# worldlife123/cbench_BaSIC

Hardware: AMD Instinct MI355X
Metric: encode+decode Mpix/s (higher is better)
Workload: dtype f32; 1 GPU; hyperprior codec N=128 M=192 (lossy_graph_scalable_exp_hp), synthetic 3x256x256 images (image i = manual_seed(i), rand), 256 images per GPU per step resident in HBM, compress+decompress incl. bitstream D2H/H2D, 6 concurrent stream workers per GPU (step k on worker k mod W: whole batches, W in flight); images_per_gpu=256, workers=6, rans_waves_per_workgroup=8, batches_in_flight=6, parallelism=image-sharded x1, RCCL all-reduce of metric sums

## Files before the change

cbench_basic_amd/_lib.py:

```python
import ctypes
import os

_HERE = os.path.dirname(os.path.abspath(__file__))
LIB_PATH = os.path.join(_HERE, "libbasic_hip.so")

OK, ERR_INVALID, ERR_NOT_INIT, ERR_HIP, ERR_OVERFLOW, ERR_NO_DEVICE = 0, -1, -2, -3, -4, -5
IMAGE_CHW, IMAGE_HWC = 0, 1
PIXEL_U8, PIXEL_F32 = 0, 1


class BasicHipError(RuntimeError):
    pass


class BasicHipInvalid(BasicHipError, ValueError):
    """A call the library refuses (BASIC_ERR_INVALID / BASIC_ERR_NOT_INIT): a ValueError, as the reference's pybind11 layer
    raises, and like every other failure of the library a BasicHipError."""


_lib = None

c_i32p = ctypes.c_void_p
_I, _L, _P, _F = ctypes.c_int, ctypes.c_int64, ctypes.c_void_p, ctypes.c_float

# ... 39 lines not shown
    "basic_rans_cost_table_host": (_I, [_P, _I, _I, _P, _I, _P]),
    "basic_rans_tables_costs": (_I, [_P, _P]),
    "basic_gc_rate_curve_dev": (_I, [_P, _P, _I, _L, _I, _P, _I, _I, _P, _I, _F, _P, _P, _P]),
    "basic_gc_quantize_index_ms_dev": (_I, [_P, _P, _P, _L, _L, _L, _P, _I, _P, _I, _F, _P, _P, _P, _P]),
    "basic_gc_dequantize_ms_dev": (_I, [_P, _P, _L, _L, _L, _P, _I, _P, _P]),
    "basic_gc_rate_curve_ms_dev": (_I, [_P, _P, _P, _L, _I, _L, _I, _P, _I, _I, _P, _I, _F, _P, _P, _P]),
    "basic_rate_select_dev": (_I, [_P, _I, _I, _L, _P, _I, _I, _P, _P, _P, _P, _P, _P]),
    "basic_rate_refine_dev": (_I, [_P, _I, _I, _P, _I, _P, _P, _P]),
    "basic_rate_select_groups_dev": (_I, [_P, _I, _I, _I, _P, _P, _P, _I, _P, _P, _P, _P, _I, _I, _P, _P, _P, _P, _P, _P, _I, _P]),
    "basic_hp_session_set_rate_targets": (_I, [_P, _P, _I, _P, _I, _I]),
    "basic_hp_session_rate_result": (_I, [_P, _P, _P, _P, _I]),
    "basic_eb_quantize_index_dev": (_I, [_P, _P, _I, _I, _I, _P, _P, _P, _P]),
    "basic_eb_dequantize_dev": (_I, [_P, _P, _I, _I, _I, _P, _P]),
    "basic_i32_to_f32_dev": (_I, [_P, _L, _P, _P]),
    "basic_pgm_gauss_encode_group_dev": (_I, [_P, _P, _I, _I, _I, _P, _L, _P, _I, _P, _P, _L, _L, _P, _P]),
    "basic_pgm_gauss_index_group_dev": (_I, [_P, _I, _I, _I, _P, _L, _P, _I, _P, _L, _L, _P]),
    "basic_pgm_gauss_scatter_group_dev": (_I, [_P, _P, _I, _I, _I, _P, _L, _L, _L, _P, _P]),
    "basic_gauss_nll_per_image_dev": (_I, [_P, _P, _I, _I, _I, _I, _F, _F, _P, _P]),
    "basic_gauss_nll_per_image_q_dev": (_I, [_P, _P, _I, _I, _I, _P, _I, _F, _F, _P, _P]),
    "basic_eb_nll_per_image_dev": (_I, [_P, _P, _I, _I, _I, _F, _P, _P]),
    "basic_conv_plan_create": (_I, [_P, _P, _I, _I, _I, _I, _I, _I, _I, _I, _P, _P, _I, _I, _P]),
    "basic_conv_plan_out_hw": (_I, [_P, _I, _I, _P, _P]),
    "basic_conv_forward_dev": (_I, [_P, _P, _I, _I, _I, _P, _P]),
    "basic_conv_plan_channels": (_I, [_P, _P, _P]),
    "basic_hp_session_create": (_I, [_P, _I, _P, _I, _P, _I, _P, _I, _P, _I, _P, _P, _I, _F, _P, _P]),
    "basic_hp_encode_bound": (_L, [_P, _I, _I, _I]),
    "basic_hp_encode_images": (_I, [_P, _P, _I, _I, _I, _I, _P, _L, _P, _P]),
    "basic_hp_encode_result": (_I, [_P, _P, _L, _P]),
    "basic_hp_decoded_shape": (_I, [_P, _P, _L, _P, _P, _P, _P]),
    "basic_hp_decode_images": (_I, [_P, _P, _L, _P, _L, _P]),
    "basic_image_u8_to_f32_dev": (_I, [_P, _I, _I, _I, _I, _I, _P, _P]),
    "basic_image_f32_to_u8_dev": (_I, [_P, _I, _I, _I, _I, _I, _P, _P]),
    "basic_image_sse_u8_dev": (_I, [_P, _I, _P, _I, _I, _I, _I, _I, _P, _P]),
    "basic_image_tiles_u8_to_f32_dev": (_I, [_P, _I, _I, _I, _I, _I, _I, _I, _I, _I, _I, _I, _I, _P, _P]),
    "basic_image_tiles_f32_to_u8_dev": (_I, [_P, _I, _I, _I, _I, _I, _I, _I, _I, _I, _I, _I, _P, _I, _I, _I, _P]),
    "basic_image_tiles_overlap_u8_to_f32_dev": (_I, [_P, _I, _I, _I, _I, _I, _I, _I, _I, _I, _I, _I, _I, _P, _P]),
    "basic_image_tiles_blend_dev": (_I, [_P, _I, _I, _I, _I, _I, _I, _I, _I, _I, _I, _I, _P, _I, _I, _P]),
    "basic_image_tiles_last_path": (_I, [_P]),
    "basic_image_tiles_gather_u8_to_f32_dev": (_I, [_P, _I, _I, _I, _I, _P, _P, _P]),
    "basic_image_tiles_scatter_f32_to_u8_dev": (_I, [_P, _I, _I, _I, _I, _I, _P, _I, _P, _P]),
    "basic_image_tiles_gather_pad_u8_to_f32_dev": (_I, [_P, _I, _I, _I, _I, _P, _P, _P]),
    "basic_image_tiles_scatter_clip_f32_to_u8_dev": (_I, [_P, _I, _I, _I, _I, _I, _P, _I, _P, _P]),
    "basic_hp_encode_images_u8": (_I, [_P, _P, _I, _I, _I, _I, _I, _P, _L, _P, _P]),
    "basic_hp_decode_images_u8": (_I, [_P, _P, _L, _I, _P, _I, _L, _P]),
    "basic_hp_session_set_rans_waves": (_I, [_P, _I]),
    "basic_hp_session_set_stream_lanes": (_I, [_P, _I]),
# ... 95 lines not shown
```

cbench_basic_amd/csrc/conv.hip:

```cpp
#include "common.h"

#include <algorithm>
#include <cmath>
#include <cstdlib>
#include <cstring>
#include <new>
#include <vector>

using namespace basic;

namespace {
thread_local bool g_dynamic_tiles = false;
}
namespace basic {
bool set_dynamic_tiles(bool on)
{
    const bool prev = g_dynamic_tiles;
    g_dynamic_tiles = on;
    return prev;
}
}

namespace {

// ... 401 lines not shown

__global__ __launch_bounds__(256) void image_absmax_kernel(const float *x, int64_t n, int per_img, unsigned *amax)
{
    const int img = blockIdx.x / per_img, part = blockIdx.x - img * per_img;
    const float *src = x + img * n;
    unsigned m = 0;
    if (((reinterpret_cast<uintptr_t>(src) | static_cast<uintptr_t>(n * 4)) & 15) == 0) {
        const u32x4 *s4 = reinterpret_cast<const u32x4 *>(src);
        for (int64_t i = part * 256 + threadIdx.x; i < n / 4; i += per_img * 256) {
            const u32x4 v = s4[i];
#pragma unroll
            for (int e = 0; e < 4; ++e) m = max(m, v[e] & 0x7FFFFFFFu);
        }
    } else {
        for (int64_t i = part * 256 + threadIdx.x; i < n; i += per_img * 256) m = max(m, __float_as_uint(src[i]) & 0x7FFFFFFFu);
    }
#pragma unroll
    for (int off = 32; off > 0; off >>= 1) m = max(m, static_cast<unsigned>(__shfl_xor(static_cast<int>(m), off)));
    if ((threadIdx.x & 63) == 0 && m) atomicMax(amax + img, m);
}

constexpr int kSplitPatchPos = 416;
constexpr int kSplitPieceBytes = kSplitPatchPos * 32;
constexpr size_t kSplitLdsPatchBytes = kSplitLdsBytes + 2 * kSplitPieceBytes;
static_assert(kSplitLdsPatchBytes <= 160 * 1024, "patch beside the weight stages");
static_assert(kSplitLdsBytes % 16 == 0, "16-byte aligned patch");
constexpr int kSplitPatchRounds = (2 * kSplitPatchPos + kSplitThreads - 1) / kSplitThreads;

template <int KH, int KW, int KWB, bool PATCH>
__global__ __launch_bounds__(kSplitThreads, 1) void conv_split_f16_kernel(const TapLaunch g, const u32x4 *wsplit, const int *kw,
                                                                          const unsigned *amax)
{
    constexpr int MT = 4;
    constexpr int kTapsA = KH * KW, kTapsAll = KH * (KW + KWB);
    constexpr int kGroups = kTapsAll / kSplitStageTaps;
    static_assert(kTapsAll % kSplitStageTaps == 0, "taps per channel block must be whole stages");
    static_assert(KWB > 0 && KWB <= KW, "fused phases: second grid inside the first");
    extern __shared__ u32x4 lds_u4[];
    float *chan_const = reinterpret_cast<float *>(lds_u4 + 2 * kSplitStageU4);

    const int tid = threadIdx.x;
    const int lane = tid & 63;
    const int khalf = lane >> 5;
    const int wave = __builtin_amdgcn_readfirstlane(tid >> 6);

    int bid = xcd_tile(blockIdx.x, gridDim.x);
    const int tx_i = bid % g.tiles_x; bid /= g.tiles_x;
    const int ty_i = bid % g.tiles_y; bid /= g.tiles_y;
    const int TB = 1 << g.tb_log, TH = 1 << g.th_log, TW = 1 << g.tw_log;
    const int b0 = bid * TB, my0 = ty_i * TH, mx0 = tx_i * TW;
    struct Pos { int tb, my, mx; };
    auto pos_of = [&](int t) {
        const int qq = (t >> 6) * 32 + (t & 31);
        return Pos{qq >> (g.tw_log + g.th_log), my0 + ((qq >> g.tw_log) & (TH - 1)), mx0 + (qq & (TW - 1))};
// ... 62 lines not shown
    if constexpr (PATCH) {
#pragma unroll
        for (int r = 0; r < kSplitPatchRounds; ++r) {
            const int i = r * kSplitThreads + tid, p = i >> 1, h = i & 1;
            const int prow = p / PW, x = p - prow * PW, img = prow / PH, row = prow - img * PH;
            const int gy = my0 + g.dymin + row, gx = mx0 + g.dxmin + x;
            const bool inside = i < 2 * npos && img < nimg && gy >= 0 && gy < g.in_h && gx >= 0 && gx < g.in_w;
            pvoff[r] = inside ? static_cast<int>((((static_cast<int64_t>(img) * g.cin + 8 * h) * g.in_h + gy) * g.in_w + gx) * 4)
                              : 0x7FFFFFF0;
            pkx[r] = inside ? split_act_exp(amax[b0 + img]) : 0;
        }
#pragma unroll
        for (int dy = 0; dy < KH; ++dy) brow[dy] = ((tb * PH + (lp.my - my0) + dy) * PW + (lp.mx - mx0)) * 32 + 16 * khalf;
    }
    float pf[kSplitPatchRounds][8];
    auto fetch_patch = [&](int cb) __attribute__((always_inline)) {
        const int soff = cb * kSplitCK * plane_bytes;
#pragma unroll
        for (int r = 0; r < kSplitPatchRounds; ++r)
#pragma unroll
            for (int j = 0; j < 8; ++j)
                pf[r][j] = __builtin_bit_cast(float, __builtin_amdgcn_raw_buffer_load_b32(rsrc, pvoff[r], soff + j * plane_bytes, 0));
    };
    auto store_patch = [&]() __attribute__((always_inline)) {
#pragma unroll
        for (int r = 0; r < kSplitPatchRounds; ++r)
            if (r * kSplitThreads + tid < 2 * npos) {
                u32x4 q[2];
                split_f16x2(pf[r], pkx[r], q[0], q[1]);
#pragma unroll
                for (int pc = 0; pc < 2; ++pc)
                    *reinterpret_cast<u32x4 *>(patch + (r * kSplitThreads + tid) * 16 + pc * kSplitPieceBytes) = q[pc];
            }
    };
    auto read_b = [&](int T, u32x4 (&d)[2]) __attribute__((always_inline)) {
        const char *src = patch + brow[tap_row(T)] + 32 * tap_col(T);
#pragma unroll
        for (int pc = 0; pc < 2; ++pc) d[pc] = *reinterpret_cast<const u32x4 *>(src + pc * kSplitPieceBytes);
    };

    f32x16 acc[MT], acc2[MT];
#pragma unroll
    for (int m = 0; m < MT; ++m)
#pragma unroll
        for (int r = 0; r < 16; ++r) {
            acc[m][r] = 0.f;
            acc2[m][r] = 0.f;
        }

    float xb[8];
    u32x4 bq[2][2];
    if constexpr (PATCH) fetch_patch(0);
    else load_b(0, 0, xb);
    fetch_w(0, 0);
    store_w(0, 0);
    fetch_w(0, 1);
    store_w(0, 1);
    if constexpr (PATCH) store_patch();
    for (int cb = 0; cb < ncb; ++cb) {
#pragma unroll
        for (int gi = 0; gi < kGroups; ++gi) {
            const int s = cb * kGroups + gi;
            __syncthreads();
            const bool more = s + 1 < ncb * kGroups;
            if (more) fetch_w(s + 1, 0);
            __builtin_amdgcn_sched_barrier(0);
            const u32x4 *wl = lds_u4 + (s & 1) * kSplitStageU4 + lane;
#pragma unroll
            for (int tl = 0; tl < kSplitStageTaps; ++tl) {
                const int T = gi * kSplitStageTaps + tl;
                float xn[8];
                u32x4 bd[2];
                if constexpr (PATCH) {
                    if (T == 0) read_b(0, bq[0]);
                } else {
                    if (T + 1 < kTapsAll) load_b(cb, T + 1, xn);
                    else load_b(cb + 1 < ncb ? cb + 1 : cb, 0, xn);
                    __builtin_amdgcn_sched_barrier(0);
                    split_f16x2(xb, kx_l, bd[0], bd[1]);
                }
                const u32x4 (&bp)[2] = PATCH ? bq[T & 1] : bd;
// ... 14 lines not shown
                        if (m == MT - 3 && T + 1 < kTapsAll) read_b(T + 1, bq[(T + 1) & 1]);
                    }
                    __builtin_amdgcn_sched_barrier(0);
                    dst[m] = mfma_f16(ap[cur][1], bp[0], dst[m]);
                    dst[m] = mfma_f16(ap[cur][0], bp[1], dst[m]);
                    dst[m] = mfma_f16(ap[cur][0], bp[0], dst[m]);
                    __builtin_amdgcn_sched_barrier(0);
                }
                if constexpr (!PATCH) {
#pragma unroll
                    for (int j = 0; j < 8; ++j) xb[j] = xn[j];
                }
                if (tl == 1 && more) {
                    store_w((s + 1) & 1, 0);
                    fetch_w(s + 1, 1);
                    __builtin_amdgcn_sched_barrier(0);
                }
                if constexpr (PATCH) {
                    if (gi == 0 && tl == 1) {
                        fetch_patch(cb + 1 < ncb ? cb + 1 : cb);
                        __builtin_amdgcn_sched_barrier(0);
                    }
                }
                if (tl == 3 && more) store_w((s + 1) & 1, 1);
            }
        }
        if constexpr (PATCH) {
            if (cb + 1 < ncb) {
                __syncthreads();
                store_patch();
            }
        }
    }

    const int tid_e = wave * 64 + static_cast<int>(__lane_id());
    const int khalf_e = (tid_e >> 5) & 1, col_e = tid_e & 31;
    float *gl = reinterpret_cast<float *>(lds_u4);
    const bool gdn = g.act == BASIC_ACT_GDN || g.act == BASIC_ACT_IGDN;
    const int be_s = b0 + pos_of(tid_e).tb;
    const int kx_e = be_s < g.batch ? split_act_exp(amax[be_s]) : 0;
    auto finish = [&](f32x16 (&acc)[MT]) __attribute__((always_inline)) {
#pragma unroll
        for (int m = 0; m < MT; ++m)
#pragma unroll
            for (int rq = 0; rq < 4; ++rq) {
                const i32x4 k4 = *reinterpret_cast<const i32x4 *>(chan_const + 256 + 32 * m + 8 * rq + 4 * khalf_e);
#pragma unroll
                for (int e = 0; e < 4; ++e) acc[m][4 * rq + e] = __builtin_ldexpf(acc[m][4 * rq + e], -(k4[e] + kx_e));
            }
        if (g.bias) {
#pragma unroll
            for (int m = 0; m < MT; ++m)
#pragma unroll
                for (int rq = 0; rq < 4; ++rq) {
// ... 26 lines not shown
                    const f32x4 b4 = *reinterpret_cast<const f32x4 *>(chan_const + 128 + 32 * m + 8 * rq + 4 * khalf_e);
#pragma unroll
                    for (int e = 0; e < 4; ++e) {
                        const int r = 4 * rq + e;
                        const float nv = nrm[m][r] + b4[e];
                        acc[m][r] *= (g.act == BASIC_ACT_GDN) ? __builtin_amdgcn_rsqf(nv) : __builtin_amdgcn_sqrtf(nv);
                    }
                }
        }
    };
    if (gdn) {
        __syncthreads();
        const f32x4 *src = reinterpret_cast<const f32x4 *>(g.gammaT);
        f32x4 *dst = reinterpret_cast<f32x4 *>(gl);
#pragma unroll
        for (int sl = 0; sl < 128 * 32 * 4 / 4 / kSplitThreads; ++sl) dst[sl * kSplitThreads + tid_e] = src[sl * kSplitThreads + tid_e];
        __syncthreads();
    }
    finish(acc);
    finish(acc2);

    const Pos ep = pos_of(tid_e);
    const int my = ep.my, mx = ep.mx, be = b0 + ep.tb;
    if (my < g.mh && mx < g.mw && be < g.batch) {
        const int oy = my * g.s_out + g.oy0, ox = mx * g.s_out + g.ox0;
        const int64_t oplane = static_cast<int64_t>(g.out_h) * g.out_w;
        float *o = g.out + (static_cast<int64_t>(be) * g.out_ctotal + g.co_base) * oplane + static_cast<int64_t>(oy) * g.out_w + ox;
#pragma unroll
        for (int m = 0; m < MT; ++m)
#pragma unroll
            for (int r = 0; r < 16; ++r) {
                const int co = 32 * m + 8 * (r >> 2) + 4 * khalf_e + (r & 3);
                if (co < g.cout) {
                    f32x2 v2;
                    v2[0] = apply_act(acc[m][r], g.act);
                    v2[1] = apply_act(acc2[m][r], g.act);
                    *reinterpret_cast<f32x2 *>(o + co * oplane) = v2;
                }
            }
    }
}

template <int KH, bool PATCH>
hipError_t launch_split(const TapLaunch &g, const u32x4 *ws, const int *kw, const unsigned *amax, int blocks, hipStream_t st)
{
    const hipError_t e = ensure_max_lds(reinterpret_cast<const void *>(conv_split_f16_kernel<KH, 3, 2, PATCH>));
    if (e != hipSuccess) return e;
    hipLaunchKernelGGL((conv_split_f16_kernel<KH, 3, 2, PATCH>), dim3(blocks), dim3(kSplitThreads),
                       PATCH ? kSplitLdsPatchBytes : kSplitLdsBytes, st, g, ws, kw, amax);
    return hipGetLastError();
}

constexpr int kFirstSlots = 10;

template <bool ROWS>
__global__ __launch_bounds__(512, 1) void conv5x5_cin4_gdn_persistent_kernel(const TapLaunch g, int ntiles, int *sched)
{
    extern __shared__ float lds[];
    constexpr int MT = 4, kCK = ROWS ? 3 : 4, KW = 5, kSteps = ROWS ? 5 * 8 : 25 * 2;
    constexpr int kWFloats = ROWS ? 80 * 32 * 4 : 25 * 4 * 32 * 4;
    constexpr int kGFloats = 128 * 32 * 4;
    float *wl = lds;
    float *gl = lds + kWFloats;
    const int tid = threadIdx.x;
    const int lane = tid & 63;
    const int wave = __builtin_amdgcn_readfirstlane(tid >> 6);
    const int khalf = lane >> 5, col = lane & 31;
    const int TB = 1 << g.tb_log, TH = 1 << g.th_log, TW = 1 << g.tw_log;
    const int chan_stride = g.ph * g.pwp;
    const int patch_elems = TB * kCK * chan_stride;
    const int patch_pad = (patch_elems + 511) / 512 * 512;
    const int n_pslots = patch_pad / 512;
// ... 949 lines not shown
    const bool two_strips = dma_ok && in_h >= 64;
    const int tile_h = two_strips ? SmTile<2>::kTileH : SmTile<1>::kTileH;
    g.tiles_y = (in_h + tile_h - 1) / tile_h;
    g.tiles_x = (in_w + kSmTileW - 1) / kSmTileW;
    const dim3 grid(batch * g.tiles_y * g.tiles_x);
    if (two_strips) hipLaunchKernelGGL(deconv5s2_cout3_dma_kernel<2>, grid, dim3(256), 0, st, g);
    else if (dma_ok) hipLaunchKernelGGL(deconv5s2_cout3_dma_kernel<1>, grid, dim3(256), 0, st, g);
    else hipLaunchKernelGGL(deconv5s2_cout3_kernel, grid, dim3(256), 0, st, g);
    BASIC_HIP_TRY(hipGetLastError());
    return BASIC_OK;
}
}

extern "C" int basic_conv_plan_launches(const basic_conv_plan *p, int batch, int in_h, int in_w)
{
    int oh = 0, ow = 0;
    if (!p || batch < 1 || basic_conv_plan_out_hw(p, in_h, in_w, &oh, &ow)) return -1;
    if (p->d_wsm) return 1;
    int n = 0;
    for_each_launch(p, choose_launches(p, batch, oh, ow, nullptr), oh, ow, [&](const Chunk &, const Phase &, int, int) { ++n; return BASIC_OK; });
    return n;
}

extern "C" int basic_conv_forward_dev(const basic_conv_plan *p, const float *d_in, int batch, int in_h, int in_w,
                                      float *d_out, void *hip_stream)
{
    BASIC_REQUIRE(p && d_in && d_out && batch >= 1, "conv_forward: bad argument");
    int oh = 0, ow = 0;
    int rc = basic_conv_plan_out_hw(p, in_h, in_w, &oh, &ow);
    if (rc) return rc;
    if (p->d_wsm) return launch_small_deconv(p, d_in, batch, in_h, in_w, d_out, as_stream(hip_stream));
    const LaunchChoice choice = choose_launches(p, batch, oh, ow, d_out);
    bool amax_done = false;
    return for_each_launch(p, choice, oh, ow, [&](const Chunk &ch, const Phase &ph, int mh, int mw) -> int {
        TapLaunch g{};
        g.in = d_in; g.out = d_out; g.wpack = ph.d_wpack; g.wrow = ph.d_wrow; g.split_wstride = ph.split_wstride; g.bias = ch.d_bias; g.gammaT = p->d_gammaT; g.beta = p->d_beta;
        g.batch = batch; g.cin = p->cin; g.cin_pad = ph.ntaps ? ph.cin_pad : 0; g.cout = ch.cout; g.coutp = ch.coutp; g.out_ctotal = p->cout; g.co_base = ch.co0;
        g.in_h = in_h; g.in_w = in_w; g.out_h = oh; g.out_w = ow;
        g.s_in = p->s_in; g.s_out = p->s_out; g.oy0 = ph.oy0; g.ox0 = ph.ox0;
        g.mh = mh; g.mw = mw;
        g.ntaps = ph.ntaps; g.dymin = ph.dymin; g.dxmin = ph.dxmin;
        std::memcpy(g.dy, ph.dy, sizeof(g.dy));
        std::memcpy(g.dx, ph.dx, sizeof(g.dx));
        g.act = p->act;
        const int kCK = ph.ck;
        if (choice.split_f16 && ph.d_wsplit) {
            const TileShape ts = tile_shape(g.mh, g.mw, kSplitWaves * 32);
            const int tw = ts.tw, th = ts.th, tb = ts.tb;
            if (static_cast<int64_t>(tb) * p->cin * in_h * in_w * 4 < (1ll << 31)) {
                g.tw_log = ilog2(tw); g.th_log = ilog2(th); g.tb_log = ilog2(tb);
                g.tiles_y = (g.mh + th - 1) / th;
                g.tiles_x = (g.mw + tw - 1) / tw;
                const int blocks = ((batch + tb - 1) / tb) * g.tiles_y * g.tiles_x;
                hipStream_t st = as_stream(hip_stream);
                const u32x4 *ws = static_cast<const u32x4 *>(ph.d_wsplit);
                BASIC_REQUIRE(ph.kw == 3 && ph.kwb == 2 && (ph.kh == 3 || ph.kh == 2), "conv_forward: split-fp16 plan / kernel instantiation mismatch");
                if (!amax_done) {
                    auto *pm = const_cast<basic_conv_plan *>(p);
                    if (pm->amax_cap < batch) {
                        if (pm->d_amax) BASIC_HIP_TRY(hipFree(pm->d_amax));
                        pm->d_amax = nullptr; pm->amax_cap = 0;
                        BASIC_HIP_TRY(hipMalloc(&pm->d_amax, sizeof(unsigned) * batch));
                        pm->amax_cap = batch;
                    }
                    BASIC_HIP_TRY(hipMemsetAsync(pm->d_amax, 0, sizeof(unsigned) * batch, st));
                    const int64_t n = static_cast<int64_t>(p->cin) * in_h * in_w;
                    const int per_img = static_cast<int>(std::min<int64_t>(64, std::max<int64_t>(1, n / 4096)));
                    hipLaunchKernelGGL(image_absmax_kernel, dim3(batch * per_img), dim3(256), 0, st, d_in, n, per_img, pm->d_amax);
                    BASIC_HIP_TRY(hipGetLastError());
                    amax_done = true;
                }
                const bool patch = choice.split_patch && g.s_in == 1 && tb * (th + ph.kh - 1) * (tw + ph.kw - 1) <= kSplitPatchPos;
                const unsigned *am = p->d_amax;
                const hipError_t e = ph.kh == 3 ? (patch ? launch_split<3, true>(g, ws, ph.d_wsplit_k, am, blocks, st) : launch_split<3, false>(g, ws, ph.d_wsplit_k, am, blocks, st))
                                                : (patch ? launch_split<2, true>(g, ws, ph.d_wsplit_k, am, blocks, st) : launch_split<2, false>(g, ws, ph.d_wsplit_k, am, blocks, st));
                BASIC_HIP_TRY(e);
                return BASIC_OK;
            }
        }
        const int threads = 64 * ph.waves, tile_pos = 32 * ph.waves;
        const TileShape ts = tile_shape(g.mh, g.mw, tile_pos);
        const int tw = ts.tw;
        int th = ts.th, tb = ts.tb;
        const bool first_layer_path = ch.mt == 4 && ch.nsplit == 1 && ph.waves == 8 && ph.kh == 5 && ph.kw == 5 &&
                                      ph.cin_pad == kCK && kCK == 4 && ch.cout == 128 && p->d_gammaT;
        g.ph = (th - 1) * g.s_in + ph.span_y;
        g.pw = (tw - 1) * g.s_in + ph.span_x;
        g.patch4 = (ph.waves == 8 && !first_layer_path && in_w % 4 == 0 && (reinterpret_cast<uintptr_t>(d_in) & 15) == 0) ? 1 : 0;
        g.pwp = g.patch4 ? (g.pw + 3 + 3) / 4 * 4 : (g.pw | 1);
        int punit = g.patch4 ? 4 : 1;
        const int mtp = mtile_pitch(ch.mt);
        const int wl_floats = g.ntaps * kCK * 32 * mtp, gam_floats = 32 * 32 * mtp;
        const int wl_pad = ((wl_floats > gam_floats ? wl_floats : gam_floats) + 4 * threads - 1) / (4 * threads) * (4 * threads);
        auto patch_slots_needed = [&](int tbv) { return (tbv * kCK * g.ph * g.pwp / punit + threads - 1) / threads; };
        auto lds_need = [&](int tbv) {
            const int patch_pad = ((tbv * kCK * g.ph * g.pwp / punit + 63) & ~63) * punit;
            return sizeof(float) * (2 * static_cast<size_t>(wl_pad + patch_pad) + 32 + 2 * g.coutp);
        };
        const int slots_avail = ph.kwb ? kPSlotsFused : patch_slots(ch.mt);
        auto too_large = [&](int tbv) { return patch_slots_needed(tbv) > slots_avail || lds_need(tbv) > 160 * 1024; };
        while (tb > 1 && too_large(tb)) tb >>= 1;
// ... 65 lines not shown
```

cbench_basic_amd/csrc/session.hip:

```cpp
#include "common.h"

#include <cstring>
#include <map>
#include <mutex>
#include <vector>

using namespace basic;

constexpr int kMaxTokenLanes = 4;


namespace {

struct DBuf {
    void *p = nullptr;
    size_t cap = 0;
    int ensure(size_t bytes)
    {
        if (bytes <= cap) return BASIC_OK;
        if (p) (void)hipFree(p);
        p = nullptr;
        cap = 0;
        const size_t want = bytes + bytes / 4 + 256;
        BASIC_HIP_TRY(hipMalloc(&p, want));
// ... 73 lines not shown
struct basic_hp_session {
    std::vector<const basic_conv_plan *> g_a, h_a, h_s, g_s;
    const basic_rans_tables *z_tables = nullptr, *y_tables = nullptr;
    int z_channels = 0, y_channels = 0, x_channels = 0, out_channels = 0, n_scales = 0;
    float scale_bound = 0.11f;
    bool mean_scale = false;
    int rans_waves = 0;
    int lanes = 1;
    int res_lanes = 1;
    std::vector<float> qsteps;
    HBuf h_steps;
    DBuf d_steps;
    hipEvent_t steps_done = nullptr;
    std::vector<int64_t> rate_budget;
    std::vector<float> rate_cand;
    int rate_passes = 0, rate_res_batch = 0;
    HBuf h_rate, h_rate_out;
    DBuf d_rate_in, d_rate_bits, d_rate_cand[2], d_rate_out;
    hipEvent_t rate_up = nullptr;
    int skip_rows = 0;
    DBuf skip_scratch, y_symc, y_idxc;
    DBuf d_medians, d_table;
    DBuf act[2], d_x, d_y, d_z, d_zhat, d_prior, d_scales;
    DBuf z_sym, z_idx, y_sym, y_idx, seg_z, seg_y, slots_z, slots_y, nw, off, packed, words, woff, state, pos;
    HBuf h_nw, h_words, h_in;
    std::vector<int64_t> off_z, off_y;
    int res_batch = 0, res_zh = 0, res_zw = 0, res_yh = 0, res_yw = 0;
    hipEvent_t in_done = nullptr;
    hipStream_t side = nullptr;
    hipEvent_t fork = nullptr, join = nullptr;
    bool use_token = false;
    int token_lanes = 0;
    hipEvent_t enc_phase = nullptr, dec_phase = nullptr;
    hipStream_t copy = nullptr;
    hipEvent_t x_free = nullptr, x_ready = nullptr;
    bool x_read_pending = false;
    DBuf u8_in, u8_out, d_xhat;
    hipEvent_t u8_free = nullptr, xhat_free = nullptr;
    bool u8_read_pending = false, xhat_read_pending = false;
    ~basic_hp_session();
};

namespace {

int run_chain(basic_hp_session *s, const std::vector<const basic_conv_plan *> &plans, const float *d_in, int batch, int h, int w,
              DBuf *out_buf, float *d_final, int *oh_out, int *ow_out, hipStream_t st)
{
    const float *cur = d_in;
    int flip = 0;
    for (size_t i = 0; i < plans.size(); ++i) {
        int oh = 0, ow = 0, co = 0;
        int rc = basic_conv_plan_out_hw(plans[i], h, w, &oh, &ow);
        if (rc) return rc;
        rc = basic_conv_plan_channels(plans[i], nullptr, &co);
        if (rc) return rc;
        const size_t bytes = sizeof(float) * static_cast<size_t>(batch) * co * oh * ow;
        float *dst;
        if (i + 1 == plans.size()) {
            if (d_final) dst = d_final;
            else { rc = out_buf->ensure(bytes); if (rc) return rc; dst = out_buf->as<float>(); }
        } else {
            rc = s->act[flip].ensure(bytes);
            if (rc) return rc;
            dst = s->act[flip].as<float>();
            flip ^= 1;
        }
        rc = basic_conv_forward_dev(plans[i], cur, batch, h, w, dst, st);
        if (rc) return rc;
        cur = dst;
        h = oh;
        w = ow;
    }
    if (oh_out) *oh_out = h;
    if (ow_out) *ow_out = w;
    return BASIC_OK;
}

int chain_out_hw(const std::vector<const basic_conv_plan *> &plans, int h, int w, int *oh, int *ow)
{
    for (const auto *p : plans) {
        int a = 0, b = 0;
        int rc = basic_conv_plan_out_hw(p, h, w, &a, &b);
        if (rc) return rc;
        h = a;
        w = b;
    }
    *oh = h;
    *ow = w;
    return BASIC_OK;
}

// ... 829 lines not shown
```

cbench_basic_amd/nn/kernels.py:

```python
import contextlib
import ctypes
import os

import numpy as np
import torch

from .. import _lib

ACT_NONE, ACT_RELU, ACT_LEAKY_RELU, ACT_GDN, ACT_IGDN = 0, 1, 2, 3, 4


def _dev(t, dtype=None):
    if not isinstance(t, torch.Tensor) or not t.is_cuda:
        raise _lib.BasicHipError("cbench_basic_amd kernels need tensors on the MI355X (got a CPU tensor); "
                                 "there is no CPU fallback")
    if dtype is not None and t.dtype != dtype:
        raise TypeError(f"expected {dtype}, got {t.dtype}")
    return t.contiguous()


def _stream():
    return torch.cuda.current_stream().cuda_stream


# ... 23 lines not shown
            int(output_padding), int(self.transposed), int(act), g.ctypes.data if g is not None else None,
            be.ctypes.data if be is not None else None, self.cin, self.cout, ctypes.byref(h)))
        self._h = h

    def __del__(self):
        h, self._h = getattr(self, "_h", None), None
        if h:
            try:
                _lib.lib().basic_conv_plan_destroy(h)
            except Exception:
                pass

    def out_hw(self, h, w):
        oh, ow = ctypes.c_int(), ctypes.c_int()
        _lib.check(_lib.lib().basic_conv_plan_out_hw(self._h, int(h), int(w), ctypes.byref(oh), ctypes.byref(ow)))
        return oh.value, ow.value

    def flops(self, batch, h, w):
        return int(_lib.lib().basic_conv_plan_flops(self._h, int(batch), int(h), int(w)))

    def launches(self, batch, h, w):
        return int(_lib.lib().basic_conv_plan_launches(self._h, int(batch), int(h), int(w)))

    def __call__(self, x, out=None):
        x = _dev(x, torch.float32)
        B, C, H, W = x.shape
        if C != self.cin:
            raise ValueError(f"conv plan expects {self.cin} input channels, got {C}")
        oh, ow = self.out_hw(H, W)
        if out is None:
            out = torch.empty((B, self.cout, oh, ow), device=x.device, dtype=torch.float32)
        _lib.check(_lib.lib().basic_conv_forward_dev(self._h, x.data_ptr(), B, H, W, out.data_ptr(), _stream()))
        return out


MCONV_KERNEL_NONE, MCONV_KERNEL_GATHER, MCONV_KERNEL_BLOCK, MCONV_KERNEL_DMA = -1, 0, 1, 2


def mconv_choose(cin, cout, ksize, in_groups, out_groups, batch, h, w, n_pos):
    k = ctypes.c_int(MCONV_KERNEL_NONE)
    _lib.check(_lib.lib().basic_mconv_choose(int(cin), int(cout), int(ksize), int(in_groups), int(out_groups), int(batch), int(h),
                                             int(w), int(n_pos), ctypes.byref(k)))
    return k.value


class MaskedConvPlan:

    def __init__(self, weight, bias, in_groups, out_groups, allow_same, act=ACT_NONE):
        w = _f32(weight)
        b = _f32(bias) if bias is not None else None
        self.cout, self.cin, self.k = w.shape[0], w.shape[1], w.shape[2]
        h = ctypes.c_void_p()
        _lib.check(_lib.lib().basic_mconv_plan_create(w.ctypes.data, b.ctypes.data if b is not None else None, self.cin,
                                                      self.cout, self.k, int(in_groups), int(out_groups), int(bool(allow_same)),
                                                      int(act), ctypes.byref(h)))
        self._h = h
# ... 1248 lines not shown
```

cbench_basic_amd/nn/models/google.py:

```python
import torch
import torch.nn as nn

from ..layers.gdn import GDN
from .. import kernels as K


def conv(in_channels, out_channels, kernel_size=5, stride=2):
    return nn.Conv2d(in_channels, out_channels, kernel_size=kernel_size, stride=stride, padding=kernel_size // 2)


def deconv(in_channels, out_channels, kernel_size=5, stride=2):
    return nn.ConvTranspose2d(in_channels, out_channels, kernel_size=kernel_size, stride=stride,
                              output_padding=stride - 1, padding=kernel_size // 2)


def compile_sequential(seq, cin_active=None, cout_actives=None):
    layers = list(seq)
    plans, i = [], 0
    while i < len(layers):
        m = layers[i]
        if not isinstance(m, (nn.Conv2d, nn.ConvTranspose2d)):
            raise TypeError(f"transform must start a fused group with a convolution, got {type(m).__name__}")
        act, gamma, beta = K.ACT_NONE, None, None
        if i + 1 < len(layers):
# ... 24 lines not shown
    def __init__(self):
        super().__init__()
        self._plans = None
        self._plan_key = None

    def _key(self):
        return tuple((p.data_ptr(), p._version) for p in self.parameters())

    def plans(self):
        key = self._key()
        if self._plans is None or key != self._plan_key:
            self._plans = compile_sequential(self.model)
            self._plan_key = key
        return self._plans

    def flops(self, batch, h, w):
        total = 0
        for p in self.plans():
            total += p.flops(batch, h, w)
            h, w = p.out_hw(h, w)
        return total

    def _forward(self, x):
        for p in self.plans():
            x = p(x)
        return x

    def forward(self, input, in_channel_gains=None, out_channel_gains=None, **kwargs):
        if in_channel_gains is not None:
            input = input * in_channel_gains.reshape(1, -1, 1, 1)
        output = self._forward(input)
        if out_channel_gains is not None:
            output = output * out_channel_gains.reshape(1, -1, 1, 1)
        return output


class HyperpriorAnalysisModel(BasicHyperpriorModule):
    def __init__(self, N, M, in_channels=3, **kwargs):
        super().__init__()
        self.in_channels, self.N, self.M = in_channels, N, M
        self.model = nn.Sequential(conv(in_channels, N), GDN(N), conv(N, N), GDN(N), conv(N, N), GDN(N), conv(N, M))


class HyperpriorSynthesisModel(BasicHyperpriorModule):
    def __init__(self, N, M, out_channels=3, **kwargs):
        super().__init__()
        self.out_channels, self.N, self.M = out_channels, N, M
        self.model = nn.Sequential(deconv(M, N), GDN(N, inverse=True), deconv(N, N), GDN(N, inverse=True),
                                   deconv(N, N), GDN(N, inverse=True), deconv(N, out_channels))
# ... 35 lines not shown
```

include/basic_hip.h:

```cpp
#ifndef BASIC_HIP_H
#define BASIC_HIP_H

#include <stdint.h>

#ifdef __cplusplus
extern "C" {
#endif

#define BASIC_OK 0
#define BASIC_ERR_INVALID (-1)
#define BASIC_ERR_NOT_INIT (-2)
#define BASIC_ERR_HIP (-3)
#define BASIC_ERR_OVERFLOW (-4)
#define BASIC_ERR_NO_DEVICE (-5)

const char *basic_last_error(void);
int basic_device_count(int *count);
int basic_set_device(int ordinal);
int basic_stream_synchronize(void *hip_stream);

typedef struct basic_rans_tables basic_rans_tables;

int basic_pmf_to_quantized_cdf(const float *pmf, int n, int precision, int32_t *cdf_out );

// ... 140 lines not shown
                                  int interleaved_mean_scale, float scale_bound, float likelihood_bound, float *d_nll,
                                  void *hip_stream);
int basic_gauss_nll_per_image_q_dev(const float *d_q, const float *d_scales, int batch, int channels, int hw, const float *d_steps,
                                    int n_steps, float scale_bound, float likelihood_bound, float *d_nll, void *hip_stream);
int basic_eb_nll_per_image_dev(const float *d_zq, const float *d_coef, int batch, int channels, int hw,
                               float likelihood_bound, float *d_nll, void *hip_stream);

typedef struct basic_conv_plan basic_conv_plan;

#define BASIC_ACT_NONE 0
#define BASIC_ACT_RELU 1
#define BASIC_ACT_LEAKY_RELU 2
#define BASIC_ACT_GDN 3
#define BASIC_ACT_IGDN 4

int basic_conv_plan_create(const float *weight, const float *bias, int cin, int cout, int ksize, int stride,
                           int padding, int output_padding, int transposed, int activation,
                           const float *gamma, const float *beta, int cin_active, int cout_active,
                           basic_conv_plan **out);
int basic_conv_plan_out_hw(const basic_conv_plan *p, int in_h, int in_w, int *out_h, int *out_w);
int basic_conv_plan_channels(const basic_conv_plan *p, int *cin_active, int *cout_active);
int basic_conv_forward_dev(const basic_conv_plan *p, const float *d_in, int batch, int in_h, int in_w,
                           float *d_out, void *hip_stream);
void basic_conv_plan_destroy(basic_conv_plan *p);
int64_t basic_conv_plan_flops(const basic_conv_plan *p, int batch, int in_h, int in_w);
int basic_conv_plan_launches(const basic_conv_plan *p, int batch, int in_h, int in_w);

typedef struct basic_mconv_plan basic_mconv_plan;
int basic_mconv_plan_create(const float *weight, const float *bias, int cin, int cout, int ksize,
                            int in_groups, int out_groups, int allow_same_topogroup, int activation,
                            basic_mconv_plan **out);
int basic_mconv_forward_pos_dev(const basic_mconv_plan *p, const float *d_x, const int32_t *d_topo_in,
                                const int32_t *d_topo_out, int batch, int h, int w, const int32_t *d_pos,
                                int64_t n_pos, float *d_y, int out_channels_total, int out_channel_offset,
                                void *hip_stream);
int basic_mconv_forward_step_dev(const basic_mconv_plan *p, const float *d_x, const int32_t *d_topo_in,
                                 const int32_t *d_topo_out, int batch, int h, int w, const int32_t *d_pos,
                                 int64_t n_pos, float *d_y, int out_channels_total, int out_channel_offset,
                                 int step, const int32_t *d_first_step, void *hip_stream);
int basic_mconv_forward_ex_dev(const basic_mconv_plan *p, const float *d_x, const int32_t *d_topo_in,
                               const int32_t *d_topo_out, int batch, int h, int w, const int32_t *d_pos, int64_t n_pos,
                               float *d_y, int out_channels_total, int out_channel_offset, int use_step, int step,
                               const int32_t *d_first_step, const int32_t *d_in_perm, const int32_t *d_out_perm,
                               void *hip_stream);
#define BASIC_MCONV_KERNEL_NONE (-1)
#define BASIC_MCONV_KERNEL_GATHER 0
// ... 172 lines not shown
```

Before: 883.4 Mpix/s.

## Fuse per-image absmax into split-fp16 conv epilogue and double-buffer patch LDS

```diff
diff --git a/cbench_basic_amd/_lib.py b/cbench_basic_amd/_lib.py
--- a/cbench_basic_amd/_lib.py
+++ b/cbench_basic_amd/_lib.py
@@ -85,6 +85,8 @@
     "basic_conv_plan_create": (_I, [_P, _P, _I, _I, _I, _I, _I, _I, _I, _I, _P, _P, _I, _I, _P]),
     "basic_conv_plan_out_hw": (_I, [_P, _I, _I, _P, _P]),
     "basic_conv_forward_dev": (_I, [_P, _P, _I, _I, _I, _P, _P]),
+    "basic_conv_forward_amax_dev": (_I, [_P, _P, _I, _I, _I, _P, _P, _P, _P]),
+    "basic_conv_plan_split_f16": (_I, [_P, _I, _I, _I, _P]),
     "basic_conv_plan_channels": (_I, [_P, _P, _P]),
     "basic_hp_session_create": (_I, [_P, _I, _P, _I, _P, _I, _P, _I, _P, _I, _P, _P, _I, _F, _P, _P]),
     "basic_hp_encode_bound": (_L, [_P, _I, _I, _I]),
diff --git a/cbench_basic_amd/csrc/conv.hip b/cbench_basic_amd/csrc/conv.hip
--- a/cbench_basic_amd/csrc/conv.hip
+++ b/cbench_basic_amd/csrc/conv.hip
@@ -447,14 +447,15 @@
 
 constexpr int kSplitPatchPos = 416;
 constexpr int kSplitPieceBytes = kSplitPatchPos * 32;
-constexpr size_t kSplitLdsPatchBytes = kSplitLdsBytes + 2 * kSplitPieceBytes;
+constexpr int kSplitPatchBufBytes = 2 * kSplitPieceBytes;
+constexpr size_t kSplitLdsPatchBytes = kSplitLdsBytes + 2 * kSplitPatchBufBytes;
 static_assert(kSplitLdsPatchBytes <= 160 * 1024, "patch beside the weight stages");
 static_assert(kSplitLdsBytes % 16 == 0, "16-byte aligned patch");
 constexpr int kSplitPatchRounds = (2 * kSplitPatchPos + kSplitThreads - 1) / kSplitThreads;
 
 template <int KH, int KW, int KWB, bool PATCH>
 __global__ __launch_bounds__(kSplitThreads, 1) void conv_split_f16_kernel(const TapLaunch g, const u32x4 *wsplit, const int *kw,
-                                                                          const unsigned *amax)
+                                                                          const unsigned *amax, unsigned *amax_out)
 {
     constexpr int MT = 4;
     constexpr int kTapsA = KH * KW, kTapsAll = KH * (KW + KWB);
@@ -563,7 +564,8 @@
             for (int j = 0; j < 8; ++j)
                 pf[r][j] = __builtin_bit_cast(float, __builtin_amdgcn_raw_buffer_load_b32(rsrc, pvoff[r], soff + j * plane_bytes, 0));
     };
-    auto store_patch = [&]() __attribute__((always_inline)) {
+    auto store_patch = [&](int buf) __attribute__((always_inline)) {
+        char *dst = patch + buf * kSplitPatchBufBytes + tid * 16;
 #pragma unroll
         for (int r = 0; r < kSplitPatchRounds; ++r)
             if (r * kSplitThreads + tid < 2 * npos) {
@@ -571,7 +573,7 @@
                 split_f16x2(pf[r], pkx[r], q[0], q[1]);
 #pragma unroll
                 for (int pc = 0; pc < 2; ++pc)
-                    *reinterpret_cast<u32x4 *>(patch + (r * kSplitThreads + tid) * 16 + pc * kSplitPieceBytes) = q[pc];
+                    *reinterpret_cast<u32x4 *>(dst + r * kSplitThreads * 16 + pc * kSplitPieceBytes) = q[pc];
             }
     };
     auto read_b = [&](int T, u32x4 (&d)[2]) __attribute__((always_inline)) {
@@ -597,7 +599,7 @@
     store_w(0, 0);
     fetch_w(0, 1);
     store_w(0, 1);
-    if constexpr (PATCH) store_patch();
+    if constexpr (PATCH) store_patch(0);
     for (int cb = 0; cb < ncb; ++cb) {
 #pragma unroll
         for (int gi = 0; gi < kGroups; ++gi) {
@@ -658,14 +660,19 @@
                         __builtin_amdgcn_sched_barrier(0);
                     }
                 }
+                if constexpr (PATCH) {
+                    if (gi == 1 && tl == 2 && cb + 1 < ncb) {
+                        store_patch((cb + 1) & 1);
+                        __builtin_amdgcn_sched_barrier(0);
+                    }
+                }
                 if (tl == 3 && more) store_w((s + 1) & 1, 1);
             }
         }
         if constexpr (PATCH) {
-            if (cb + 1 < ncb) {
-                __syncthreads();
-                store_patch();
-            }
+            const int flip = (cb & 1) ? -kSplitPatchBufBytes : kSplitPatchBufBytes;
+#pragma unroll
+            for (int dy = 0; dy < KH; ++dy) brow[dy] += flip;
         }
     }
 
@@ -738,6 +745,7 @@
 
     const Pos ep = pos_of(tid_e);
     const int my = ep.my, mx = ep.mx, be = b0 + ep.tb;
+    unsigned omax = 0;
     if (my < g.mh && mx < g.mw && be < g.batch) {
         const int oy = my * g.s_out + g.oy0, ox = mx * g.s_out + g.ox0;
         const int64_t oplane = static_cast<int64_t>(g.out_h) * g.out_w;
@@ -752,18 +760,28 @@
                     v2[0] = apply_act(acc[m][r], g.act);
                     v2[1] = apply_act(acc2[m][r], g.act);
                     *reinterpret_cast<f32x2 *>(o + co * oplane) = v2;
-                }
-            }
+                    omax = max(omax, max(__float_as_uint(v2[0]) & 0x7FFFFFFFu, __float_as_uint(v2[1]) & 0x7FFFFFFFu));
+                }
+            }
+    }
+    if (amax_out) {
+        const int img_lanes = (TH * TW < 32) ? TH * TW : 32;
+        omax = max(omax, static_cast<unsigned>(__shfl_xor(static_cast<int>(omax), 32)));
+#pragma unroll
+        for (int off = 16; off > 0; off >>= 1)
+            if (off < img_lanes) omax = max(omax, static_cast<unsigned>(__shfl_xor(static_cast<int>(omax), off)));
+        if ((tid_e & 32) == 0 && (tid_e & (img_lanes - 1)) == 0 && omax) atomicMax(amax_out + be, omax);
     }
 }
 
 template <int KH, bool PATCH>
-hipError_t launch_split(const TapLaunch &g, const u32x4 *ws, const int *kw, const unsigned *amax, int blocks, hipStream_t st)
+hipError_t launch_split(const TapLaunch &g, const u32x4 *ws, const int *kw, const unsigned *amax, unsigned *amax_out, int blocks,
+                        hipStream_t st)
 {
     const hipError_t e = ensure_max_lds(reinterpret_cast<const void *>(conv_split_f16_kernel<KH, 3, 2, PATCH>));
     if (e != hipSuccess) return e;
     hipLaunchKernelGGL((conv_split_f16_kernel<KH, 3, 2, PATCH>), dim3(blocks), dim3(kSplitThreads),
-                       PATCH ? kSplitLdsPatchBytes : kSplitLdsBytes, st, g, ws, kw, amax);
+                       PATCH ? kSplitLdsPatchBytes : kSplitLdsBytes, st, g, ws, kw, amax, amax_out);
     return hipGetLastError();
 }
 
@@ -1759,16 +1777,64 @@
     return n;
 }
 
+namespace {
+bool launch_is_split_f16(const basic_conv_plan *p, const LaunchChoice &c, const Phase &ph, int mh, int mw, int in_h, int in_w)
+{
+    if (!c.split_f16 || !ph.d_wsplit) return false;
+    const TileShape ts = tile_shape(mh, mw, kSplitWaves * 32);
+    return static_cast<int64_t>(ts.tb) * p->cin * in_h * in_w * 4 < (1ll << 31);
+}
+
+int queue_image_absmax(const float *d_x, int batch, int64_t n, unsigned *amax, hipStream_t st)
+{
+    BASIC_HIP_TRY(hipMemsetAsync(amax, 0, sizeof(unsigned) * batch, st));
+    const int per_img = static_cast<int>(std::min<int64_t>(64, std::max<int64_t>(1, n / 4096)));
+    hipLaunchKernelGGL(image_absmax_kernel, dim3(batch * per_img), dim3(256), 0, st, d_x, n, per_img, amax);
+    BASIC_HIP_TRY(hipGetLastError());
+    return BASIC_OK;
+}
+}
+
+extern "C" int basic_conv_plan_split_f16(const basic_conv_plan *p, int batch, int in_h, int in_w, const float *d_out)
+{
+    int oh = 0, ow = 0;
+    if (!p || batch < 1 || basic_conv_plan_out_hw(p, in_h, in_w, &oh, &ow)) return -1;
+    if (p->d_wsm) return 0;
+    int n = 0, nsplit = 0;
+    const LaunchChoice choice = choose_launches(p, batch, oh, ow, d_out);
+    for_each_launch(p, choice, oh, ow, [&](const Chunk &, const Phase &ph, int mh, int mw) {
+        ++n;
+        nsplit += launch_is_split_f16(p, choice, ph, mh, mw, in_h, in_w) ? 1 : 0;
+        return BASIC_OK;
+    });
+    return n > 0 && nsplit == n ? 1 : 0;
+}
+
 extern "C" int basic_conv_forward_dev(const basic_conv_plan *p, const float *d_in, int batch, int in_h, int in_w,
                                       float *d_out, void *hip_stream)
 {
+    return basic_conv_forward_amax_dev(p, d_in, batch, in_h, in_w, d_out, nullptr, nullptr, hip_stream);
+}
+
+extern "C" int basic_conv_forward_amax_dev(const basic_conv_plan *p, const float *d_in, int batch, int in_h, int in_w,
+                                           float *d_out, const unsigned *d_amax_in, unsigned *d_amax_out, void *hip_stream)
+{
     BASIC_REQUIRE(p && d_in && d_out && batch >= 1, "conv_forward: bad argument");
+    BASIC_REQUIRE(!d_amax_out || d_amax_out != d_amax_in, "conv_forward: amax_out must not be amax_in");
     int oh = 0, ow = 0;
     int rc = basic_conv_plan_out_hw(p, in_h, in_w, &oh, &ow);
     if (rc) return rc;
+    const bool amax_fused = d_amax_out && basic_conv_plan_split_f16(p, batch, in_h, in_w, d_out) == 1;
+    if (d_amax_out && !amax_fused) {
+        rc = p->d_wsm ? launch_small_deconv(p, d_in, batch, in_h, in_w, d_out, as_stream(hip_stream))
+                      : basic_conv_forward_amax_dev(p, d_in, batch, in_h, in_w, d_out, d_amax_in, nullptr, hip_stream);
+        if (rc) return rc;
+        return queue_image_absmax(d_out, batch, static_cast<int64_t>(p->cout) * oh * ow, d_amax_out, as_stream(hip_stream));
+    }
     if (p->d_wsm) return launch_small_deconv(p, d_in, batch, in_h, in_w, d_out, as_stream(hip_stream));
+    if (amax_fused) BASIC_HIP_TRY(hipMemsetAsync(d_amax_out, 0, sizeof(unsigned) * batch, as_stream(hip_stream)));
     const LaunchChoice choice = choose_launches(p, batch, oh, ow, d_out);
-    bool amax_done = false;
+    bool amax_done = d_amax_in != nullptr;
     return for_each_launch(p, choice, oh, ow, [&](const Chunk &ch, const Phase &ph, int mh, int mw) -> int {
         TapLaunch g{};
         g.in = d_in; g.out = d_out; g.wpack = ph.d_wpack; g.wrow = ph.d_wrow; g.split_wstride = ph.split_wstride; g.bias = ch.d_bias; g.gammaT = p->d_gammaT; g.beta = p->d_beta;
@@ -1781,39 +1847,35 @@
         std::memcpy(g.dx, ph.dx, sizeof(g.dx));
         g.act = p->act;
         const int kCK = ph.ck;
-        if (choice.split_f16 && ph.d_wsplit) {
+        if (launch_is_split_f16(p, choice, ph, mh, mw, in_h, in_w)) {
             const TileShape ts = tile_shape(g.mh, g.mw, kSplitWaves * 32);
             const int tw = ts.tw, th = ts.th, tb = ts.tb;
-            if (static_cast<int64_t>(tb) * p->cin * in_h * in_w * 4 < (1ll << 31)) {
-                g.tw_log = ilog2(tw); g.th_log = ilog2(th); g.tb_log = ilog2(tb);
-                g.tiles_y = (g.mh + th - 1) / th;
-                g.tiles_x = (g.mw + tw - 1) / tw;
-                const int blocks = ((batch + tb - 1) / tb) * g.tiles_y * g.tiles_x;
-                hipStream_t st = as_stream(hip_stream);
-                const u32x4 *ws = static_cast<const u32x4 *>(ph.d_wsplit);
-                BASIC_REQUIRE(ph.kw == 3 && ph.kwb == 2 && (ph.kh == 3 || ph.kh == 2), "conv_forward: split-fp16 plan / kernel instantiation mismatch");
-                if (!amax_done) {
-                    auto *pm = const_cast<basic_conv_plan *>(p);
-                    if (pm->amax_cap < batch) {
-                        if (pm->d_amax) BASIC_HIP_TRY(hipFree(pm->d_amax));
-                        pm->d_amax = nullptr; pm->amax_cap = 0;
-                        BASIC_HIP_TRY(hipMalloc(&pm->d_amax, sizeof(unsigned) * batch));
-                        pm->amax_cap = batch;
-                    }
-                    BASIC_HIP_TRY(hipMemsetAsync(pm->d_amax, 0, sizeof(unsigned) * batch, st));
-                    const int64_t n = static_cast<int64_t>(p->cin) * in_h * in_w;
-                    const int per_img = static_cast<int>(std::min<int64_t>(64, std::max<int64_t>(1, n / 4096)));
-                    hipLaunchKernelGGL(image_absmax_kernel, dim3(batch * per_img), dim3(256), 0, st, d_in, n, per_img, pm->d_amax);
-                    BASIC_HIP_TRY(hipGetLastError());
-                    amax_done = true;
-                }
-                const bool patch = choice.split_patch && g.s_in == 1 && tb * (th + ph.kh - 1) * (tw + ph.kw - 1) <= kSplitPatchPos;
-                const unsigned *am = p->d_amax;
-                const hipError_t e = ph.kh == 3 ? (patch ? launch_split<3, true>(g, ws, ph.d_wsplit_k, am, blocks, st) : launch_split<3, false>(g, ws, ph.d_wsplit_k, am, blocks, st))
-                                                : (patch ? launch_split<2, true>(g, ws, ph.d_wsplit_k, am, blocks, st) : launch_split<2, false>(g, ws, ph.d_wsplit_k, am, blocks, st));
-                BASIC_HIP_TRY(e);
-                return BASIC_OK;
-            }
+            g.tw_log = ilog2(tw); g.th_log = ilog2(th); g.tb_log = ilog2(tb);
+            g.tiles_y = (g.mh + th - 1) / th;
+            g.tiles_x = (g.mw + tw - 1) / tw;
+            const int blocks = ((batch + tb - 1) / tb) * g.tiles_y * g.tiles_x;
+            hipStream_t st = as_stream(hip_stream);
+            const u32x4 *ws = static_cast<const u32x4 *>(ph.d_wsplit);
+            BASIC_REQUIRE(ph.kw == 3 && ph.kwb == 2 && (ph.kh == 3 || ph.kh == 2), "conv_forward: split-fp16 plan / kernel instantiation mismatch");
+            if (!amax_done) {
+                auto *pm = const_cast<basic_conv_plan *>(p);
+                if (pm->amax_cap < batch) {
+                    if (pm->d_amax) BASIC_HIP_TRY(hipFree(pm->d_amax));
+                    pm->d_amax = nullptr; pm->amax_cap = 0;
+                    BASIC_HIP_TRY(hipMalloc(&pm->d_amax, sizeof(unsigned) * batch));
+                    pm->amax_cap = batch;
+                }
+                const int qrc = queue_image_absmax(d_in, batch, static_cast<int64_t>(p->cin) * in_h * in_w, pm->d_amax, st);
+                if (qrc) return qrc;
+                amax_done = true;
+            }
+            const bool patch = choice.split_patch && g.s_in == 1 && tb * (th + ph.kh - 1) * (tw + ph.kw - 1) <= kSplitPatchPos;
+            const unsigned *am = d_amax_in ? d_amax_in : p->d_amax;
+            unsigned *ao = amax_fused ? d_amax_out : nullptr;
+            const hipError_t e = ph.kh == 3 ? (patch ? launch_split<3, true>(g, ws, ph.d_wsplit_k, am, ao, blocks, st) : launch_split<3, false>(g, ws, ph.d_wsplit_k, am, ao, blocks, st))
+                                            : (patch ? launch_split<2, true>(g, ws, ph.d_wsplit_k, am, ao, blocks, st) : launch_split<2, false>(g, ws, ph.d_wsplit_k, am, ao, blocks, st));
+            BASIC_HIP_TRY(e);
+            return BASIC_OK;
         }
         const int threads = 64 * ph.waves, tile_pos = 32 * ph.waves;
         const TileShape ts = tile_shape(g.mh, g.mw, tile_pos);
diff --git a/cbench_basic_amd/csrc/session.hip b/cbench_basic_amd/csrc/session.hip
--- a/cbench_basic_amd/csrc/session.hip
+++ b/cbench_basic_amd/csrc/session.hip
@@ -119,6 +119,7 @@
     DBuf skip_scratch, y_symc, y_idxc;
     DBuf d_medians, d_table;
     DBuf act[2], d_x, d_y, d_z, d_zhat, d_prior, d_scales;
+    DBuf amax[2];
     DBuf z_sym, z_idx, y_sym, y_idx, seg_z, seg_y, slots_z, slots_y, nw, off, packed, words, woff, state, pos;
     HBuf h_nw, h_words, h_in;
     std::vector<int64_t> off_z, off_y;
@@ -144,7 +145,8 @@
               DBuf *out_buf, float *d_final, int *oh_out, int *ow_out, hipStream_t st)
 {
     const float *cur = d_in;
-    int flip = 0;
+    int flip = 0, aflip = 0;
+    const unsigned *amax_in = nullptr;
     for (size_t i = 0; i < plans.size(); ++i) {
         int oh = 0, ow = 0, co = 0;
         int rc = basic_conv_plan_out_hw(plans[i], h, w, &oh, &ow);
@@ -162,8 +164,17 @@
             dst = s->act[flip].as<float>();
             flip ^= 1;
         }
-        rc = basic_conv_forward_dev(plans[i], cur, batch, h, w, dst, st);
-        if (rc) return rc;
+        unsigned *amax_out = nullptr;
+        if (i + 1 < plans.size() && basic_conv_plan_split_f16(plans[i], batch, h, w, dst) == 1 &&
+            basic_conv_plan_split_f16(plans[i + 1], batch, oh, ow, nullptr) == 1) {
+            rc = s->amax[aflip].ensure(sizeof(unsigned) * batch);
+            if (rc) return rc;
+            amax_out = s->amax[aflip].as<unsigned>();
+            aflip ^= 1;
+        }
+        rc = basic_conv_forward_amax_dev(plans[i], cur, batch, h, w, dst, amax_in, amax_out, st);
+        if (rc) return rc;
+        amax_in = amax_out;
         cur = dst;
         h = oh;
         w = ow;
diff --git a/cbench_basic_amd/nn/kernels.py b/cbench_basic_amd/nn/kernels.py
--- a/cbench_basic_amd/nn/kernels.py
+++ b/cbench_basic_amd/nn/kernels.py
@@ -69,7 +69,13 @@
     def launches(self, batch, h, w):
         return int(_lib.lib().basic_conv_plan_launches(self._h, int(batch), int(h), int(w)))
 
-    def __call__(self, x, out=None):
+    def split_f16(self, batch, h, w, out=None):
+        r = int(_lib.lib().basic_conv_plan_split_f16(self._h, int(batch), int(h), int(w), out.data_ptr() if out is not None else None))
+        if r < 0:
+            raise ValueError("conv plan: bad input shape")
+        return r == 1
+
+    def __call__(self, x, out=None, amax_in=None, amax_out=None):
         x = _dev(x, torch.float32)
         B, C, H, W = x.shape
         if C != self.cin:
@@ -77,8 +83,30 @@
         oh, ow = self.out_hw(H, W)
         if out is None:
             out = torch.empty((B, self.cout, oh, ow), device=x.device, dtype=torch.float32)
-        _lib.check(_lib.lib().basic_conv_forward_dev(self._h, x.data_ptr(), B, H, W, out.data_ptr(), _stream()))
+        if amax_in is None and amax_out is None:
+            _lib.check(_lib.lib().basic_conv_forward_dev(self._h, x.data_ptr(), B, H, W, out.data_ptr(), _stream()))
+            return out
+        for a in (amax_in, amax_out):
+            if a is not None and (_dev(a, torch.int32) is not a or a.numel() != B):
+                raise ValueError("amax tensors are contiguous int32 [batch] on the device")
+        _lib.check(_lib.lib().basic_conv_forward_amax_dev(
+            self._h, x.data_ptr(), B, H, W, out.data_ptr(), amax_in.data_ptr() if amax_in is not None else None,
+            amax_out.data_ptr() if amax_out is not None else None, _stream()))
         return out
+
+
+def run_plans(plans, x):
+    amax_in = None
+    for i, p in enumerate(plans):
+        amax_out = None
+        if i + 1 < len(plans):
+            B, _, H, W = x.shape
+            oh, ow = p.out_hw(H, W)
+            if p.split_f16(B, H, W) and plans[i + 1].split_f16(B, oh, ow):
+                amax_out = torch.empty((B,), device=x.device, dtype=torch.int32)
+        x = p(x, amax_in=amax_in, amax_out=amax_out)
+        amax_in = amax_out
+    return x
 
 
 MCONV_KERNEL_NONE, MCONV_KERNEL_GATHER, MCONV_KERNEL_BLOCK, MCONV_KERNEL_DMA = -1, 0, 1, 2
diff --git a/cbench_basic_amd/nn/models/google.py b/cbench_basic_amd/nn/models/google.py
--- a/cbench_basic_amd/nn/models/google.py
+++ b/cbench_basic_amd/nn/models/google.py
@@ -70,9 +70,7 @@
         return total
 
     def _forward(self, x):
-        for p in self.plans():
-            x = p(x)
-        return x
+        return K.run_plans(self.plans(), x)
 
     def forward(self, input, in_channel_gains=None, out_channel_gains=None, **kwargs):
         if in_channel_gains is not None:
diff --git a/include/basic_hip.h b/include/basic_hip.h
--- a/include/basic_hip.h
+++ b/include/basic_hip.h
@@ -186,6 +186,9 @@
 int basic_conv_plan_channels(const basic_conv_plan *p, int *cin_active, int *cout_active);
 int basic_conv_forward_dev(const basic_conv_plan *p, const float *d_in, int batch, int in_h, int in_w,
                            float *d_out, void *hip_stream);
+int basic_conv_forward_amax_dev(const basic_conv_plan *p, const float *d_in, int batch, int in_h, int in_w,
+                                float *d_out, const unsigned *d_amax_in, unsigned *d_amax_out, void *hip_stream);
+int basic_conv_plan_split_f16(const basic_conv_plan *p, int batch, int in_h, int in_w, const float *d_out);
 void basic_conv_plan_destroy(basic_conv_plan *p);
 int64_t basic_conv_plan_flops(const basic_conv_plan *p, int batch, int in_h, int in_w);
 int basic_conv_plan_launches(const basic_conv_plan *p, int batch, int in_h, int in_w);
```

Result: no change. 882.6 Mpix/s, median of 2 (-0.1%).
